# bastienjossen/DDL25Spring

Hardware: AMD Instinct MI355X
Metric: FedAvg rounds/sec + local samples/sec, ResNet-18 CIFAR-10-shape, 8 clients (higher is better)
Workload: dtype fp32; 1 GPU; model=resnet18-cifar10, global_batch=800, parallelism=fedavg-8clients-dp1, clients=8, local_batch=100, local_epochs=1, samples_per_client=6250, client_slots_per_gpu=8, hip_graphs=True, fp32_conv_math=auto

## Files before the change

### csrc/kernels/conv_f32.hip

```cpp
#include "conv_f32_core.h"
#include <cstdlib>

#ifndef F32_PREFETCH
#define F32_PREFETCH 2
#endif

constexpr int FBK = 16;

__device__ __forceinline__ int fswz(int row) { return (row >> 2) & 2; }
__device__ __forceinline__ int lds_off(int row, int ch) { return row * 16 + ((ch ^ fswz(row)) << 2); }

__device__ __forceinline__ int x6_off(int row, int ch, int half) {
  const int f = row & 2;
  const int g = (row ^ (row >> 2)) & 1;
  return row * 32 + 8 * (ch ^ f) + 4 * (half ^ g);
}

template <int MODE, int BP, int BQ, int X6>
__global__ __launch_bounds__(256, (X6 && BP * BQ <= 64 * 128) ? 3 : 2) void convf32_kernel(ConvF32Args a) {
  constexpr int WP = BP / 2, WQ = BQ / 2, TP = WP / 16, TQ = WQ / 16;
  constexpr int RW = X6 ? 32 : 16;
  constexpr int SP = BP * RW, SQ = BQ * RW;
  constexpr int UPK = BP / 64, UQK = BQ / 64;
  constexpr int KUP = BP / 64, KUQ = BQ / 64;
  __shared__ float4 smem4[(2 * (SP + SQ)) / 4];
  float* smem = (float*)smem4;
  __shared__ float xform[2 * 512];

  const int tid = threadIdx.x, lane = tid & 63, wid = tid >> 6, wp = wid >> 1, wq = wid & 1;
  const int gx = gridDim.x, gy = gridDim.y, gz = gridDim.z;
  const int lin = blockIdx.x + gx * (blockIdx.y + gy * blockIdx.z);
  const int u = xcd_remap(lin, gx * gy * gz);
  const int bx = u % gx, by = (u / gx) % gy, g = u / (gx * gy);
  const FGeo o = fgeo<MODE, BP, BQ>(a, bx, by, g, gy);
  const bool split_store = a.split_k > 1;
  if (o.q0 >= o.Qd || o.p0 >= o.Pd) {
    if (!split_store || (a.tickets && o.split == 0)) fzero_slot<MODE, BP>(a, o);
    return;
  }
  const int nk = (o.Kr + FBK - 1) / FBK;
  const int per = (nk + o.nsplit - 1) / o.nsplit;
  const int kt0 = o.split * per, kt1 = min(nk, kt0 + per);

  const int H = a.H, W = a.W, C = a.C, K = a.K, S = a.S, P = a.P, Q = a.Q, st = a.stride, pd = a.pad;
  const float* X = a.x + (long long)g * a.x_gs;
  const float* Wt = a.w + (long long)g * a.w_gs;
  const float* DY = a.dy + (long long)g * a.dy_gs;
  const bool xf = (MODE != F_DGRAD) && a.in_scale != nullptr;
  if (xf) {
    for (int i = tid; i < C; i += 256) {
      xform[i] = a.in_scale[(long long)g * C + i];
      xform[512 + i] = a.in_shift[(long long)g * C + i];
    }
  }
  const bool xrelu = a.in_relu != 0;

  int pk_row[UPK], pk_ch[UPK];
  int pm_rg = 0, pm_kp = 0;
  if constexpr (MODE == F_FWD) {
#pragma unroll
    for (int i = 0; i < UPK; ++i) {
      const int uu = tid + 256 * i;
      pk_row[i] = uu >> 2;
      pk_ch[i] = uu & 3;
    }
  } else {
    pm_kp = tid % (16 / KUP);
    pm_rg = tid / (16 / KUP);
  }
  int qk_row[UQK], qk_ch[UQK], qk_n[UQK], qk_hb[UQK], qk_wb[UQK];
  int qm_rg = 0, qm_kp = 0, qm_r = 0, qm_s = 0, qm_c = 0;
  bool qm_ok = false;
  float qm_sc[4] = {1.f, 1.f, 1.f, 1.f}, qm_sh[4] = {0.f, 0.f, 0.f, 0.f};
  if constexpr (MODE != F_WGRAD) {
    const FDiv dpq = mk_fdiv((uint32_t)(MODE == F_FWD ? P * Q : o.Hs * o.Ws));
    const FDiv dq = mk_fdiv((uint32_t)(MODE == F_FWD ? Q : o.Ws));
    const int PQ = MODE == F_FWD ? P * Q : o.Hs * o.Ws, QQ = MODE == F_FWD ? Q : o.Ws;
#pragma unroll
    for (int i = 0; i < UQK; ++i) {
      const int uu = tid + 256 * i;
      qk_row[i] = uu >> 2;
      qk_ch[i] = uu & 3;
      const int q = o.q0 + qk_row[i];
      if (q < o.Qd) {
        const int n = fdv(q, dpq), rem = q - n * PQ;
        const int y = fdv(rem, dq), xq = rem - y * QQ;
        qk_n[i] = n;
        if (MODE == F_FWD) {
          qk_hb[i] = y * st - pd;
          qk_wb[i] = xq * st - pd;
        } else {
          qk_hb[i] = (o.nph == 4 ? 2 * y + o.pa : y) + pd;
          qk_wb[i] = (o.nph == 4 ? 2 * xq + o.pb : xq) + pd;
        }
      } else {
        qk_n[i] = -1;
        qk_hb[i] = qk_wb[i] = 0;
      }
    }
  } else {
    qm_kp = tid % (16 / KUQ);
    qm_rg = tid / (16 / KUQ);
    const int q = o.q0 + 4 * qm_rg;
    qm_ok = q < o.Qd;
    if (qm_ok) {
      const int tap = q / C;
      qm_c = q - tap * C;
      qm_r = tap / S;
      qm_s = tap - qm_r * S;
    }
  }
  if (xf) __syncthreads();
  if constexpr (MODE == F_WGRAD) {
    if (xf && qm_ok) {
#pragma unroll
      for (int v = 0; v < 4; ++v) { qm_sc[v] = xform[qm_c + v]; qm_sh[v] = xform[512 + qm_c + v]; }
    }
  }
  const FDiv dpix = mk_fdiv((uint32_t)(P * Q)), dpq1 = mk_fdiv((uint32_t)Q);

  constexpr unsigned OOB = 0xFFFFFFF0u;
  const __amdgpu_buffer_rsrc_t rX = __builtin_amdgcn_make_buffer_rsrc(
      (void*)X, 0, (int)((long long)a.N * H * W * C * 4), 0x00020000);
  const __amdgpu_buffer_rsrc_t rW = __builtin_amdgcn_make_buffer_rsrc(
      (void*)Wt, 0, (int)((long long)K * a.R * S * C * 4), 0x00020000);
  const __amdgpu_buffer_rsrc_t rD = __builtin_amdgcn_make_buffer_rsrc(
      (void*)DY, 0, (int)((long long)a.N * P * Q * K * 4), 0x00020000);
  auto bload = [&](const __amdgpu_buffer_rsrc_t& rs, unsigned off) -> float4 {
    const auto v = __builtin_amdgcn_raw_buffer_load_b128(rs, off, 0, 0);
    return __builtin_bit_cast(float4, v);
  };
  constexpr int PF = F32_PREFETCH;
  float4 rpA[2], rqA[2], rpB[2], rqB[2], rpC[2], rqC[2];
  bool qvA[2] = {false, false}, qvB[2] = {false, false}, qvC[2] = {false, false};
  auto load_step = [&](int kt, float4 (&rp)[2], float4 (&rq)[2], bool (&qv)[2]) {
    const int kk0 = kt * FBK;
    if constexpr (MODE == F_FWD) {
#pragma unroll
      for (int i = 0; i < UPK; ++i) {
        const int p = o.p0 + pk_row[i];
        rp[i] = bload(rW, p < o.Pd ? (unsigned)(p * o.Kr + kk0 + 4 * pk_ch[i]) * 4u : OOB);
      }
    } else if constexpr (MODE == F_DGRAD) {
      const int tap = kk0 / K, k0 = kk0 - tap * K;
      const int ir = tap / o.Sn, is = tap - ir * o.Sn;
      const int r = o.r0 + (st == 2 ? 2 : 1) * ir, s = o.s0 + (st == 2 ? 2 : 1) * is;
      const int c = o.p0 + 4 * pm_rg;
#pragma unroll
      for (int j = 0; j < KUP; ++j) {
        const int k = k0 + pm_kp * KUP + j;
        rp[j] = bload(rW, c < C ? (unsigned)(((k * a.R + r) * S + s) * C + c) * 4u : OOB);
      }
    } else {
      const int kch = o.p0 + 4 * pm_rg;
#pragma unroll
      for (int j = 0; j < KUP; ++j) {
        const int pix = kk0 + pm_kp * KUP + j;
        rp[j] = bload(rD, (pix < o.Kr && kch < K) ? (unsigned)(pix * K + kch) * 4u : OOB);
      }
    }
    if constexpr (MODE == F_FWD) {
      const int tap = kk0 / C, c0 = kk0 - tap * C;
      const int r = tap / S, s = tap - r * S;
#pragma unroll
      for (int i = 0; i < UQK; ++i) {
        const int h = qk_hb[i] + r, w = qk_wb[i] + s;
        const bool ok = qk_n[i] >= 0 && (unsigned)h < (unsigned)H && (unsigned)w < (unsigned)W;
        qv[i] = ok;
        rq[i] = bload(rX, ok ? (unsigned)(((qk_n[i] * H + h) * W + w) * C + c0 + 4 * qk_ch[i]) * 4u : OOB);
      }
    } else if constexpr (MODE == F_DGRAD) {
      const int tap = kk0 / K, k0 = kk0 - tap * K;
      const int ir = tap / o.Sn, is = tap - ir * o.Sn;
      const int r = o.r0 + (st == 2 ? 2 : 1) * ir, s = o.s0 + (st == 2 ? 2 : 1) * is;
#pragma unroll
      for (int i = 0; i < UQK; ++i) {
        int ho = qk_hb[i] - r, wo = qk_wb[i] - s;
        bool hit = true;
        if (st == 2) {
          ho >>= 1;
          wo >>= 1;
        } else if (st > 2) {
          hit = ho >= 0 && wo >= 0 && ho % st == 0 && wo % st == 0;
          ho /= st;
          wo /= st;
        }
        const bool ok = hit && qk_n[i] >= 0 && (unsigned)ho < (unsigned)P && (unsigned)wo < (unsigned)Q;
        rq[i] = bload(rD, ok ? (unsigned)(((qk_n[i] * P + ho) * Q + wo) * K + k0 + 4 * qk_ch[i]) * 4u : OOB);
      }
    } else {
#pragma unroll
      for (int j = 0; j < KUQ; ++j) {
        const int pix = kk0 + qm_kp * KUQ + j;
        const int n = fdv(pix, dpix), rem = pix - n * P * Q;
        const int ho = fdv(rem, dpq1), wo = rem - ho * Q;
        const int h = ho * st - pd + qm_r, w = wo * st - pd + qm_s;
        const bool ok = qm_ok && pix < o.Kr && (unsigned)h < (unsigned)H && (unsigned)w < (unsigned)W;
        qv[j] = ok;
        rq[j] = bload(rX, ok ? (unsigned)(((n * H + h) * W + w) * C + qm_c) * 4u : OOB);
      }
    }
  };
  auto xform4 = [&](float4 v, const float* sc, const float* sh) {
    v.x = v.x * sc[0] + sh[0];
    v.y = v.y * sc[1] + sh[1];
    v.z = v.z * sc[2] + sh[2];
    v.w = v.w * sc[3] + sh[3];
    if (xrelu) { v.x = fmaxf(v.x, 0.f); v.y = fmaxf(v.y, 0.f); v.z = fmaxf(v.z, 0.f); v.w = fmaxf(v.w, 0.f); }
    return v;
  };
  auto store_mn = [&](float* img, int rg, int kp, int KU, const float4* v) {
#pragma unroll
    for (int j4 = 0; j4 < 4; ++j4) {
      const int row = 4 * rg + j4;
      const int kk = kp * KU;
      float* d = img + row * 16 + (((kk >> 2) ^ fswz(row)) << 2) + (kk & 3);
      const float e0 = j4 == 0 ? v[0].x : j4 == 1 ? v[0].y : j4 == 2 ? v[0].z : v[0].w;
      if (KU == 2) {
        const float e1 = j4 == 0 ? v[1].x : j4 == 1 ? v[1].y : j4 == 2 ? v[1].z : v[1].w;
        *(float2*)d = make_float2(e0, e1);
      } else {
        *d = e0;
      }
    }
  };
  auto store_k6 = [&](float* img, int row, int ch, float4 v) {
    s4v h, m, l;
    split3(v, h, m, l);
    *(s8v*)(img + x6_off(row, ch, 0)) = cat44(h, m);
    *(s8v*)(img + x6_off(row, ch, 1)) = cat44(l, h);
  };
  auto store_mn6 = [&](float* img, int rg, int kp, int KU, const float4* v) {
#pragma unroll
    for (int j4 = 0; j4 < 4; ++j4) {
      const int row = 4 * rg + j4;
      const int kk = kp * KU, ch = kk >> 2, pos = kk & 3;
      uint16_t* h0 = (uint16_t*)(img + x6_off(row, ch, 0)) + pos;
      uint16_t* h1 = (uint16_t*)(img + x6_off(row, ch, 1)) + pos;
      const float e0 = j4 == 0 ? v[0].x : j4 == 1 ? v[0].y : j4 == 2 ? v[0].z : v[0].w;
      uint16_t ah, am, al;
      split1(e0, ah, am, al);
      if (KU == 2) {
        const float e1 = j4 == 0 ? v[1].x : j4 == 1 ? v[1].y : j4 == 2 ? v[1].z : v[1].w;
        uint16_t bh, bm, bl;
        split1(e1, bh, bm, bl);
        *(uint32_t*)h0 = (uint32_t)ah | ((uint32_t)bh << 16);
        *(uint32_t*)(h0 + 4) = (uint32_t)am | ((uint32_t)bm << 16);
        *(uint32_t*)h1 = (uint32_t)al | ((uint32_t)bl << 16);
        *(uint32_t*)(h1 + 4) = (uint32_t)ah | ((uint32_t)bh << 16);
      } else {
        h0[0] = ah;
        h0[4] = am;
        h1[0] = al;
        h1[4] = ah;
      }
    }
  };
  auto store_step = [&](int buf, int kt, float4 (&rp)[2], float4 (&rq)[2], const bool (&qv)[2]) {
    float* Ps = smem + buf * (SP + SQ);
    float* Qs = Ps + SP;
    if constexpr (MODE == F_FWD) {
#pragma unroll
      for (int i = 0; i < UPK; ++i) {
        if constexpr (X6) store_k6(Ps, pk_row[i], pk_ch[i], rp[i]);
        else *(float4*)(Ps + lds_off(pk_row[i], pk_ch[i])) = rp[i];
      }
    } else {
      if constexpr (X6) store_mn6(Ps, pm_rg, pm_kp, KUP, rp);
      else store_mn(Ps, pm_rg, pm_kp, KUP, rp);
    }
    if constexpr (MODE == F_FWD) {
      if (xf) {
        const int kk0 = kt * FBK, c0 = kk0 - (kk0 / C) * C;
#pragma unroll
        for (int i = 0; i < UQK; ++i) {
          const int c = c0 + 4 * qk_ch[i];
          if (qv[i]) rq[i] = xform4(rq[i], xform + c, xform + 512 + c);
        }
      }
    } else if constexpr (MODE == F_WGRAD) {
      if (xf) {
#pragma unroll
        for (int j = 0; j < KUQ; ++j)
          if (qv[j]) rq[j] = xform4(rq[j], qm_sc, qm_sh);
      }
    }
    if constexpr (MODE != F_WGRAD) {
#pragma unroll
      for (int i = 0; i < UQK; ++i) {
        if constexpr (X6) store_k6(Qs, qk_row[i], qk_ch[i], rq[i]);
        else *(float4*)(Qs + lds_off(qk_row[i], qk_ch[i])) = rq[i];
      }
    } else {
      if constexpr (X6) store_mn6(Qs, qm_rg, qm_kp, KUQ, rq);
      else store_mn(Qs, qm_rg, qm_kp, KUQ, rq);
    }
  };

  f4v acc[TP][TQ];
#pragma unroll
  for (int i = 0; i < TP; ++i)
#pragma unroll
    for (int j = 0; j < TQ; ++j) acc[i][j] = (f4v){0.f, 0.f, 0.f, 0.f};

  auto step = [&](int kt, float4 (&cp)[2], float4 (&cq)[2], bool (&cv)[2], float4 (&np)[2],
                  float4 (&nq)[2], bool (&nv)[2]) {
    const int cur = (kt - kt0) & 1;
    if (kt + PF < kt1) load_step(kt + PF, np, nq, nv);
    const float* Ps = smem + cur * (SP + SQ);
    const float* Qs = Ps + SP;
    if constexpr (X6) {
      s8v a0[TP], a1[TP], b0[TQ], b1[TQ];
#pragma unroll
      for (int ti = 0; ti < TP; ++ti) {
        const int R = wp * WP + ti * 16 + (lane & 15);
        a0[ti] = *(const s8v*)(Ps + x6_off(R, lane >> 4, 0));
        a1[ti] = *(const s8v*)(Ps + x6_off(R, lane >> 4, 1));
      }
#pragma unroll
      for (int tj = 0; tj < TQ; ++tj) {
        const int R = wq * WQ + tj * 16 + (lane & 15);
        b0[tj] = *(const s8v*)(Qs + x6_off(R, lane >> 4, 0));
        b1[tj] = *(const s8v*)(Qs + x6_off(R, lane >> 4, 1));
      }
#pragma unroll
      for (int ti = 0; ti < TP; ++ti)
#pragma unroll
        for (int tj = 0; tj < TQ; ++tj) {
          f4v c = __builtin_amdgcn_mfma_f32_16x16x32_bf16(a1[ti], b0[tj], (f4v){0.f, 0.f, 0.f, 0.f}, 0, 0, 0);
          c = __builtin_amdgcn_mfma_f32_16x16x32_bf16(a0[ti], b1[tj], c, 0, 0, 0);
          c = __builtin_amdgcn_mfma_f32_16x16x32_bf16(a0[ti], b0[tj], c, 0, 0, 0);
#pragma unroll
          for (int v = 0; v < 4; ++v) acc[ti][tj][v] = acc[ti][tj][v] + c[v];
        }
    } else {
      float4 af[TP], bfr[TQ];
#pragma unroll
      for (int ti = 0; ti < TP; ++ti)
        af[ti] = *(const float4*)(Ps + lds_off(wp * WP + ti * 16 + (lane & 15), lane >> 4));
#pragma unroll
      for (int tj = 0; tj < TQ; ++tj)
        bfr[tj] = *(const float4*)(Qs + lds_off(wq * WQ + tj * 16 + (lane & 15), lane >> 4));
#pragma unroll
      for (int s4 = 0; s4 < 4; ++s4)
#pragma unroll
        for (int ti = 0; ti < TP; ++ti)
#pragma unroll
          for (int tj = 0; tj < TQ; ++tj) {
            const float av = s4 == 0 ? af[ti].x : s4 == 1 ? af[ti].y : s4 == 2 ? af[ti].z : af[ti].w;
            const float bv = s4 == 0 ? bfr[tj].x : s4 == 1 ? bfr[tj].y : s4 == 2 ? bfr[tj].z : bfr[tj].w;
            acc[ti][tj] = __builtin_amdgcn_mfma_f32_16x16x4f32(av, bv, acc[ti][tj], 0, 0, 0);
          }
    }
    if (kt + 1 < kt1) store_step(cur ^ 1, kt + 1, cp, cq, cv);
    __syncthreads();
  };
  if (kt0 < kt1) {
    load_step(kt0, rpA, rqA, qvA);
    if (kt0 + 1 < kt1) load_step(kt0 + 1, rpB, rqB, qvB);
    if constexpr (PF == 3) {
      if (kt0 + 2 < kt1) load_step(kt0 + 2, rpC, rqC, qvC);
    }
    store_step(0, kt0, rpA, rqA, qvA);
    __syncthreads();
    if constexpr (PF == 3) {
      for (int kt = kt0; kt < kt1; kt += 3) {
        step(kt, rpB, rqB, qvB, rpA, rqA, qvA);
        if (kt + 1 < kt1) step(kt + 1, rpC, rqC, qvC, rpB, rqB, qvB);
        if (kt + 2 < kt1) step(kt + 2, rpA, rqA, qvA, rpC, rqC, qvC);
      }
    } else {
      for (int kt = kt0; kt < kt1; kt += 2) {
        step(kt, rpB, rqB, qvB, rpA, rqA, qvA);
        if (kt + 1 < kt1) step(kt + 1, rpA, rqA, qvA, rpB, rqB, qvB);
      }
    }
  }

  if (split_store) {
#pragma unroll
    for (int ti = 0; ti < TP; ++ti)
#pragma unroll
      for (int tj = 0; tj < TQ; ++tj) {
        const int q = o.q0 + wq * WQ + tj * 16 + (lane & 15);
        const int p = o.p0 + wp * WP + ti * 16 + 4 * (lane >> 4);
        if (q >= o.Qd || p >= o.Pd) continue;
        if constexpr (MODE == F_WGRAD) {
          float* d = a.partial + ((long long)o.split * a.G + g) * o.Pd * o.Qd;
#pragma unroll
          for (int v = 0; v < 4; ++v)
            if (p + v < o.Pd) d[(long long)(p + v) * o.Qd + q] = acc[ti][tj][v];
        } else {
          const long long qmax = (long long)a.slots / o.nph * BQ;
          float* d = a.partial + (((long long)o.split * a.G + g) * o.nph + o.phase) * qmax * o.Pd;
          *(float4*)(d + (long long)q * o.Pd + p) = make_float4(acc[ti][tj][0], acc[ti][tj][1],
                                                                acc[ti][tj][2], acc[ti][tj][3]);
        }
      }
    if (a.tickets) {
      __threadfence();
      __syncthreads();
      int* const last = (int*)smem;
      int* const ticket = a.tickets + ((long long)g * o.nph + o.phase) * gx + bx;
      if (tid == 0) *last = atomicAdd(ticket, 1) == o.nsplit - 1;
      __syncthreads();
      if (!*last) return;
      __threadfence();
      if constexpr (MODE != F_WGRAD) {
        const long long qmax = (long long)a.slots / o.nph * BQ;
        const long long slice = (long long)a.G * o.nph * qmax * o.Pd;
        const float* base = a.partial + ((long long)g * o.nph + o.phase) * qmax * o.Pd;
#pragma unroll
        for (int ti = 0; ti < TP; ++ti)
#pragma unroll
          for (int tj = 0; tj < TQ; ++tj) {
            const int q = o.q0 + wq * WQ + tj * 16 + (lane & 15);
            const int p = o.p0 + wp * WP + ti * 16 + 4 * (lane >> 4);
            f4v sm = (f4v){0.f, 0.f, 0.f, 0.f};
            if (q < o.Qd && p < o.Pd) {
              const float* src = base + (long long)q * o.Pd + p;
              for (int k = 0; k < o.nsplit; ++k) {
                const float4 v = *(const float4*)(src + k * slice);
                sm[0] += v.x; sm[1] += v.y; sm[2] += v.z; sm[3] += v.w;
              }
            }
            acc[ti][tj] = sm;
          }
        __syncthreads();
        if (tid == 0) *ticket = 0;
        fepi<MODE, BP, BQ, Lay16<BP, BQ>>(a, o, acc, smem);
        return;
      } else {
        const long long per = (long long)o.Pd * o.Qd;
        const float* src = a.partial + (long long)g * per;
        float* dst = a.out + (long long)g * a.out_gs;
        for (int e = tid; e < BP * (BQ / 4); e += 256) {
          const int p = o.p0 + e / (BQ / 4), q = o.q0 + 4 * (e % (BQ / 4));
          if (p >= o.Pd || q >= o.Qd) continue;
          const long long off = (long long)p * o.Qd + q;
          float4 sum = make_float4(0.f, 0.f, 0.f, 0.f);
          for (int k = 0; k < o.nsplit; ++k) {
            const float4 v = *(const float4*)(src + (long long)k * a.G * per + off);
            sum.x += v.x; sum.y += v.y; sum.z += v.z; sum.w += v.w;
          }
          float4 b = a.accumulate ? *(const float4*)(dst + off) : make_float4(0.f, 0.f, 0.f, 0.f);
          b.x += a.gscale * sum.x; b.y += a.gscale * sum.y; b.z += a.gscale * sum.z; b.w += a.gscale * sum.w;
          *(float4*)(dst + off) = b;
        }
        if (tid == 0) *ticket = 0;
      }
    }
    return;
  }
  fepi<MODE, BP, BQ, Lay16<BP, BQ>>(a, o, acc, smem);
}

template <int V>
__global__ __launch_bounds__(256) void convf32_wgrad_reduce(const float* __restrict__ part, float* out,
                                                            long long out_gs, int G, long long nv,
                                                            int splits, int accumulate, float gscale) {
  typedef float vec __attribute__((ext_vector_type(V)));
  const long long per = nv * V;
  GSTRIDE_LOOP(t, (long long)G * nv) {
    const long long g = t / nv, i = (t - g * nv) * V;
    vec s = (vec)(0.f);
    const float* src = part + g * per + i;
    const long long sstride = (long long)G * per;
    int k = 0;
    for (; k + 8 <= splits; k += 8) {
      vec v[8];
#pragma unroll
      for (int j = 0; j < 8; ++j) v[j] = *(const vec*)(src + (long long)(k + j) * sstride);
#pragma unroll
      for (int j = 0; j < 8; ++j) s += v[j];
    }
    for (; k < splits; ++k) s += *(const vec*)(src + (long long)k * sstride);
    float* d = out + g * out_gs + i;
    vec b = accumulate ? *(const vec*)d : (vec)(0.f);
    b += gscale * s;
    *(vec*)d = b;
  }
}

static void launch_wgrad_reduce(const float* part, float* out, long long out_gs, int G, long long n, int splits,
                                int accumulate, float gscale, hipStream_t s) {
  static const long long v4_min = [] {
    const char* e = getenv("DDL_WGRAD_REDUCE_V4_MIN");
    return e ? atoll(e) : 512LL * 256;
  }();
  if ((long long)G * (n / 4) >= v4_min)
    hipLaunchKernelGGL(convf32_wgrad_reduce<4>, dim3(grid_for((long long)G * (n / 4), 256)), dim3(256), 0, s, part,
                       out, out_gs, G, n / 4, splits, accumulate, gscale);
  else
    hipLaunchKernelGGL(convf32_wgrad_reduce<1>, dim3(grid_for((long long)G * n, 256)), dim3(256), 0, s, part, out,
                       out_gs, G, n, splits, accumulate, gscale);
}

DDL_API int ddl_convf32_wgrad_reduce(const float* part, float* out, long long out_gs, int G, long long n, int splits,
                                     int accumulate, float gscale, hipStream_t s) {
  if (n % 4) return (int)hipErrorInvalidValue;
  launch_wgrad_reduce(part, out, out_gs, G, n, splits, accumulate, gscale, s);
  return (int)hipGetLastError();
}

static void fdims(const ConvF32Args& a, int mode, long long& Pd, long long& Qd, long long& Qmax, long long& Kr,
                  int& nph) {
  nph = (mode == F_DGRAD && a.stride == 2) ? 4 : 1;
  if (mode == F_FWD) { Pd = a.K; Qd = Qmax = (long long)a.N * a.P * a.Q; Kr = (long long)a.R * a.S * a.C; }
  else if (mode == F_DGRAD) {
    Pd = a.C;
    const int Hs = nph == 4 ? (a.H + 1) >> 1 : a.H, Ws = nph == 4 ? (a.W + 1) >> 1 : a.W;
    Qd = Qmax = (long long)a.N * Hs * Ws;
    Kr = (long long)a.R * a.S * a.K;
  } else { Pd = a.K; Qd = Qmax = (long long)a.R * a.S * a.C; Kr = (long long)a.N * a.P * a.Q; }
}

DDL_API long long ddl_convf32_slots(const ConvF32Args* ap, int mode, int cfg) {
  long long Pd, Qd, Qmax, Kr;
  int nph;
  fdims(*ap, mode, Pd, Qd, Qmax, Kr, nph);
  const int bq = ((cfg >> 8) & 0xff) * 16;
  if (bq <= 0) return -1;
  return nph * ((Qmax + bq - 1) / bq);
}

DDL_API long long ddl_convf32_workspace(const ConvF32Args* ap, int mode, int cfg) {
  if (ap->split_k <= 1) return 0;
  long long Pd, Qd, Qmax, Kr;
  int nph;
  fdims(*ap, mode, Pd, Qd, Qmax, Kr, nph);
  const int bq = ((cfg >> 8) & 0xff) * 16;
  if (mode == F_WGRAD) return (long long)ap->split_k * ap->G * Pd * Qd;
  const long long qm = (Qmax + bq - 1) / bq * bq;
  return (long long)ap->split_k * ap->G * nph * qm * Pd;
}

template <int MODE, int BP, int BQ, int X6>
static int launch_tile(ConvF32Args a, hipStream_t s) {
  long long Pd, Qd, Qmax, Kr;
  int nph;
  fdims(a, MODE, Pd, Qd, Qmax, Kr, nph);
  const long long ntp = (Pd + BP - 1) / BP, ntq = (Qmax + BQ - 1) / BQ;
  a.slots = (int)(nph * ntq);
  const int split = a.split_k < 1 ? 1 : a.split_k;
  a.split_k = split;
  if (split > 1) {
    const long long need = MODE == F_WGRAD ? (long long)split * a.G * Pd * Qd
                                           : (long long)split * a.G * nph * ntq * BQ * Pd;
    if (!a.partial || need > a.partial_cap) return (int)hipErrorInvalidValue;
  }
  const dim3 grid((unsigned)(ntp * ntq), (unsigned)(nph * split), (unsigned)a.G);
  if (split == 1 || (long long)a.G * nph * ntp * ntq > a.tickets_cap) a.tickets = nullptr;
  hipLaunchKernelGGL((convf32_kernel<MODE, BP, BQ, X6>), grid, dim3(256), 0, s, a);
  hipError_t e = hipGetLastError();
  if (e != hipSuccess || split == 1 || a.tickets) return (int)e;
  if (MODE == F_WGRAD) {
    launch_wgrad_reduce((const float*)a.partial, a.out, a.out_gs, a.G, Pd * Qd, split, a.accumulate, a.gscale, s);
  } else {
    hipLaunchKernelGGL((convf32_splitk_epilogue<MODE, BP, BQ>), dim3((unsigned)(ntp * ntq), nph, a.G),
                       dim3(256), 0, s, a);
  }
  return (int)hipGetLastError();
}

template <int MODE, int X6>
static int launch_math(const ConvF32Args& a, int bp, int bq, hipStream_t s) {
  if (bp == 64 && bq == 64) return launch_tile<MODE, 64, 64, X6>(a, s);
  if (bp == 64 && bq == 128) return launch_tile<MODE, 64, 128, X6>(a, s);
  if (bp == 128 && bq == 64) return launch_tile<MODE, 128, 64, X6>(a, s);
  if (bp == 128 && bq == 128) return launch_tile<MODE, 128, 128, X6>(a, s);
  return (int)hipErrorInvalidValue;
}

template <int MODE>
static int launch_mode(const ConvF32Args& a, int cfg, hipStream_t s) {
  const int bp = (cfg & 0xff) * 16, bq = ((cfg >> 8) & 0xff) * 16;
  return (cfg >> 16) & 1 ? launch_math<MODE, 1>(a, bp, bq, s) : launch_math<MODE, 0>(a, bp, bq, s);
}

DDL_API int ddl_convf32(const ConvF32Args* ap, int mode, int cfg, hipStream_t s) {
  const ConvF32Args& a = *ap;
  if (a.G < 1 || a.N < 1 || a.C < 1 || a.K < 1 || a.stride < 1) return (int)hipErrorInvalidValue;
  if (a.C > 512 && a.in_scale) return (int)hipErrorInvalidValue;
  const long long lim = (1LL << 31) - 64;
  if ((long long)a.N * a.H * a.W * a.C * 4 > lim || (long long)a.K * a.R * a.S * a.C * 4 > lim ||
      (long long)a.N * a.P * a.Q * a.K * 4 > lim)
    return (int)hipErrorInvalidValue;
  if (mode == F_FWD) {
    if (a.C % 16 || a.K % 4) return (int)hipErrorInvalidValue;
    return launch_mode<F_FWD>(a, cfg, s);
  }
  if (mode == F_DGRAD) {
    if (a.K % 16 || a.C % 4) return (int)hipErrorInvalidValue;
    return launch_mode<F_DGRAD>(a, cfg, s);
  }
  if (mode == F_WGRAD) {
    if (a.C % 4 || a.K % 4) return (int)hipErrorInvalidValue;
    if (!a.accumulate && a.gscale != 1.f) return (int)hipErrorInvalidValue;
    return launch_mode<F_WGRAD>(a, cfg, s);
  }
  return (int)hipErrorInvalidValue;
}

DDL_API int ddl_convf32_args_size() { return (int)sizeof(ConvF32Args); }
```

### ddl25spring_amd/ops/functional_f32.py

```python
from __future__ import annotations

import ctypes
import math
import os

import torch

from . import _lib
from . import workspace as ws
from ._lib import check, ptr, stream

F_FWD, F_DGRAD, F_WGRAD = 0, 1, 2
WS_CAP = 1 << 26
_WS: dict = {}
TARGET_WG = int(os.environ.get("DDL_F32_TARGET_WG", "640"))


def is_f32(t) -> bool:
    return t is not None and t.is_cuda and t.dtype == torch.float32


class SlotStats:
    __slots__ = ("t", "rows")

    def __init__(self):
        self.t = None
        self.rows = 0


def workspace(device, role: str = "main") -> torch.Tensor:
    key = f"{device}:{role}"
    b = _WS.get(key)
    if b is None:
        if torch.cuda.is_current_stream_capturing():
            raise RuntimeError("fp32 split-K workspace first requested inside a graph capture: run one eager "
                               "step (or functional_f32.ensure_workspace) before capturing")
        ensure_workspace(device)
        b = _WS[key]
    return b


def ensure_workspace(device) -> None:
    for role in ("main", "side"):
        key = f"{device}:{role}"
        if key not in _WS:
            _WS[key] = torch.empty(WS_CAP, dtype=torch.float32, device=device)
            _WS[key + ":tickets"] = torch.zeros(TICKETS_CAP, dtype=torch.int32, device=device)
    if torch.device(device).type == "cuda" and _dev_key(device) not in _TICKETS:
        _TICKETS[_dev_key(device)] = torch.zeros(TICKETS_N, dtype=torch.int32, device=device)


TICKETS_CAP = 1 << 18
WG_FOLD = [os.environ.get("DDL_F32_WG_FOLD", "0") == "1"]


def _dims(mode, g):
    if mode == F_FWD:
        return g.K, g.N * g.P * g.Q, g.R * g.S * g.C, 1
    if mode == F_DGRAD:
        if g.stride == 2:
            hs, wsz = (g.H + 1) // 2, (g.W + 1) // 2
            rn, sn = (g.R + 1) // 2, (g.S + 1) // 2
            return g.C, g.N * hs * wsz, rn * sn * g.K, 4
        return g.C, g.N * g.H * g.W, g.R * g.S * g.K, 1
    return g.K, g.R * g.S * g.C, g.N * g.P * g.Q, 1


def cfg_of(bp: int, bq: int) -> int:
    return (bp // 16) | ((bq // 16) << 8)


MATHS = ("mfma32", "x6", "auto")
_MATH = [os.environ.get("DDL_F32_MATH", "auto")]
if _MATH[0] not in MATHS:
    raise ValueError(f"DDL_F32_MATH={_MATH[0]!r}: expected one of {MATHS}")


def math() -> str:
    return _MATH[0]


def set_math(name: str) -> None:
    if name not in MATHS:
        raise ValueError(f"fp32 conv math {name!r}: expected one of {MATHS}")
    if name != _MATH[0]:
        _MATH[0] = name
        _PLANS.clear()


X6_BIT = 1 << 16
HALO_BIT = 1 << 17
_HALO = [os.environ.get("DDL_F32_HALO", "1") != "0"]
HALO_HPMAX = 288


def set_halo(on: bool) -> None:
    if bool(on) != _HALO[0]:
        _HALO[0] = bool(on)
        _PLANS.clear()


HALO_MIN_W = int(os.environ.get("DDL_F32_HALO_MIN_W", "4"))
HALO_PADW = [os.environ.get("DDL_F32_HALO_PADW", "1") != "0"]


def halo_ok(mode: int, g, auto: bool = False) -> bool:
    if mode not in (F_FWD, F_DGRAD) or g.stride != 1 or g.R != g.S or g.R not in (1, 3) or g.pad != (g.R - 1) // 2:
        return False
    if g.P != g.H or g.Q != g.W:
        return False
    OH, OWr = g.P, g.Q
    if OWr < 4 or OWr > 128:
        return False
    if auto and OWr < HALO_MIN_W:
        return False
    OW = 1 << (OWr - 1).bit_length()
    if OW != OWr and (not HALO_PADW[0] or (auto and g.R == 1)):
        return False
    TR = 128 // OW
    if TR <= OH:
        if OH % TR:
            return False
        SR = TR
    else:
        if TR % OH:
            return False
        SR = OH
    HP = (TR // SR) * (SR + g.R - 1) * (OW + g.S - 1)
    SC, Pd = (g.C, g.K) if mode == F_FWD else (g.K, g.C)
    if not (HP <= HALO_HPMAX and SC % 16 == 0 and Pd % 4 == 0):
        return False
    return _x6h_native_ok(mode, g)


_X6H_OK: dict = {}


def _x6h_native_ok(mode: int, g) -> bool:
    key = (mode, g)
    r = _X6H_OK.get(key)
    if r is None:
        try:
            lib = _lib.kernels()
        except Exception:
            return True
        a = _args(g)
        r = bool(lib.ddl_x6h_ok(ctypes.byref(a), mode, cfg_of(64, 128)))
        _X6H_OK[key] = r
    return r


HALO_TINY, HALO_SMALL, HALO_LARGE = 26624, 32768, 45056


def halo_layout(mode: int, geom, bp: int = 64):
    out = (ctypes.c_int * 5)()
    a = _args(geom)
    if _lib.kernels().ddl_x6h_layout(ctypes.byref(a), mode, cfg_of(bp, 128), out) != 0:
        return None
    return dict(zip(("ROWB", "SEGB", "HBYTES", "HP", "tier"), out))


def halo_residency(mode: int, bp: int, rs: int, tier: int, padw: bool = False) -> int:
    return int(_lib.kernels().ddl_x6h_residency(mode, bp, rs, tier, int(padw)))


_FLAT_ENV = os.environ.get("DDL_F32_FLAT1X1", "fd")
FLAT1X1 = [_FLAT_ENV != "0", "fdw" if _FLAT_ENV == "1" else _FLAT_ENV]


def _launch_geom(geom, mode: str = "f"):
    if not FLAT1X1[0] or mode not in FLAT1X1[1] or geom.R != 1 or geom.S != 1 or geom.stride != 1 or geom.pad != 0:
        return geom
    if geom.W & (geom.W - 1) == 0 and geom.W <= 128:
        return geom
    npix = geom.N * geom.H * geom.W
    if npix % 128:
        return geom
    return type(geom)(geom.G, 1, npix // 128, 128, geom.C, geom.K, 1, 1, 1, 0)


def _cfg(cfg: int) -> int:
    if _MATH[0] == "x6":
        return cfg | X6_BIT
    if _MATH[0] == "mfma32":
        return cfg & ~X6_BIT
    return cfg


_PLANS: dict = {}
_OVERRIDE: dict = {}
_MODE_NAMES = ("fwd", "dgrad", "wgrad")
_TUNED_PATH = os.path.join(os.path.dirname(os.path.abspath(__file__)), "f32_plans.json")
_TUNED: dict | None = None


def _tuned(mode: int, g):
    global _TUNED
    if _TUNED is None:
        _TUNED = {}
        if os.environ.get("DDL_F32_TUNED", "1") != "0" and os.path.exists(_TUNED_PATH):
            import json
            with open(_TUNED_PATH) as f:
                _TUNED = json.load(f).get("plans", {})
    key = f"{_MODE_NAMES[mode]}:{g.G},{g.N},{g.H},{g.W},{g.C},{g.K},{g.R},{g.S},{g.stride},{g.pad}"
    if _MATH[0] == "auto":
        p = _TUNED.get(f"auto:{key}")
        if p is not None:
            return cfg_of(p[0], p[1]) | (X6_BIT if p[3] == "x6" else 0), int(p[2])
        p = _TUNED.get(f"x6:{key}")
        return None if p is None else (cfg_of(p[0], p[1]) | X6_BIT, int(p[2]))
    if _MATH[0] != "mfma32":
        key = f"{_MATH[0]}:{key}"
    p = _TUNED.get(key)
    return None if p is None else (cfg_of(p[0], p[1]), int(p[2]))


BLAS = [os.environ.get("DDL_F32_BLAS", "0")]


def vendor_gemm(mode: int, g) -> bool:
    if BLAS[0] in ("0", "1"):
        return BLAS[0] == "1"
    _tuned(mode, g)
    return f"blas:{_MODE_NAMES[mode]}:{g.G},{g.N},{g.H},{g.W},{g.C},{g.K},{g.R},{g.S},{g.stride},{g.pad}" in _TUNED


def set_plan(mode: int, geom, bp: int, bq: int, split: int, engine: str | None = None) -> None:
    bits = {None: X6_BIT, "x6": X6_BIT, "x6h": X6_BIT | HALO_BIT, "mfma32": 0}[engine]
    _OVERRIDE[(mode, geom)] = (cfg_of(bp, bq) | bits, int(split))
    _PLANS.pop((mode, geom), None)


def clear_plan(mode: int, geom) -> None:
    _OVERRIDE.pop((mode, geom), None)
    _PLANS.pop((mode, geom), None)


_RECORD_PATH = os.environ.get("DDL_F32_RECORD", "")
_RECORDED: set = set()


def _write_record():
    import json
    rows = sorted({(m, (g.G, g.N, g.H, g.W, g.C, g.K, g.R, g.S, g.stride, g.pad)) for m, g in _RECORDED})
    with open(_RECORD_PATH, "w") as f:
        json.dump([{"mode": _MODE_NAMES[m], "geom": list(g)} for m, g in rows], f)


if _RECORD_PATH:
    import atexit
    atexit.register(_write_record)


def plan(mode: int, geom) -> tuple[int, int]:
    key = (mode, geom)
    p = _PLANS.get(key)
    if p is not None:
        return p
    if _RECORD_PATH:
        _RECORDED.add(key)
    p = _OVERRIDE.get(key)
    if p is None and _HALO[0] and _MATH[0] != "mfma32" and halo_ok(mode, geom, auto=True):
        p = _halo_plan(mode, geom)
    if p is None:
        p = _tuned(mode, geom)
    if p is None:
        Pd, Qd, Kr, nph = _dims(mode, geom)
        bp = 128 if Pd > 64 else 64
        bq = 128 if Qd > 64 else 64
        tiles = -(-Pd // bp) * -(-Qd // bq) * nph * geom.G
        nk = -(-Kr // 16)
        split = 1
        while tiles * split < TARGET_WG and nk >= split * 2 * 8 and split < 64:
            split *= 2
        p = (cfg_of(bp, bq) | X6_BIT, split)
    _PLANS[key] = p
    return p


def _halo_plan(mode: int, geom) -> tuple[int, int]:
    _tuned(mode, geom)
    if TARGET_WG != 1:
        p = _TUNED.get(f"x6h:{_MODE_NAMES[mode]}:{geom.G},{geom.N},{geom.H},{geom.W},{geom.C},{geom.K},"
                       f"{geom.R},{geom.S},{geom.stride},{geom.pad}")
        if p is not None:
            return cfg_of(int(p[0]), int(p[1])) | X6_BIT | HALO_BIT, int(p[2])
    Pd, Qd, _, _ = _dims(mode, geom)
    SC = geom.C if mode == F_FWD else geom.K
    bp = 128 if Pd > 64 and geom.Q > 4 else 64
    tiles = -(-Pd // bp) * -(-Qd // 128) * geom.G
    nch = SC // 16
    split = 1
    padded = geom.Q & (geom.Q - 1) != 0
    while not padded and tiles * split < TARGET_WG and nch >= split * 2 * 4 and split < 32:
        split *= 2
    return cfg_of(bp, 128) | X6_BIT | HALO_BIT, split


def _args(geom, **kw) -> _lib.ConvF32Args:
    a = _lib.ConvF32Args()
    a.gscale = 1.0
    for k, v in kw.items():
        setattr(a, k, v)
    a.G, a.N, a.H, a.W, a.C, a.K = geom.G, geom.N, geom.H, geom.W, geom.C, geom.K
    a.R, a.S, a.P, a.Q, a.stride, a.pad = geom.R, geom.S, geom.P, geom.Q, geom.stride, geom.pad
    return a


def _gs(t) -> int:
    return 0 if t is None else t.stride(0)


def _launch(a, mode: int, geom, device, split_k: int = 0, ws_role: str = "main") -> None:
    lib = _lib.kernels()
    cfg, split = plan(mode, geom)
    if split_k:
        split = split_k
    a.split_k = split
    cfg = _cfg(cfg)
    if cfg & HALO_BIT and not halo_ok(mode, geom):
        cfg &= ~HALO_BIT
    if split > 1:
        need = lib.ddl_convf32_workspace(ctypes.byref(a), mode, cfg)
        buf = workspace(device, ws_role)
        if need > buf.numel():
            a.split_k = split = 1
        else:
            a.partial, a.partial_cap = buf.data_ptr(), buf.numel()
            if WG_FOLD[0] and not (cfg & HALO_BIT):
                t = _WS[f"{device}:{ws_role}:tickets"]
                a.tickets, a.tickets_cap = t.data_ptr(), t.numel()
    name = ("conv_fwd", "conv_dgrad", "conv_wgrad")[mode] + "_f32"
    if cfg & HALO_BIT:
        ws_buf = split_weights(a, mode, geom, device)
        a.wsplit, a.ws_gs = ws_buf.data_ptr(), ws_buf.stride(0)
        check(lib.ddl_x6h(ctypes.byref(a), mode, cfg & ~HALO_BIT, stream()), name + "_halo")
        return
    check(lib.ddl_convf32(ctypes.byref(a), mode, cfg, stream()), name)


def split_weights(a, mode: int, geom, device) -> torch.Tensor:
    T = geom.R * geom.S
    layout = 0 if mode == F_FWD else 1
    scope = _PRESPLIT[0]
    if scope is not None:
        key = (int(a.w), layout, geom.G, geom.K, T, geom.C, int(a.w_gs))
        buf = scope.lookup(key)
        if buf is not None:
            return buf
    out = torch.empty(geom.G, geom.K * T * geom.C * 6, dtype=torch.uint8, device=device)
    check(_lib.kernels().ddl_x6_split_weights(a.w, out.data_ptr(), geom.G, geom.K, T, geom.C, 0 if mode == F_FWD else 1,
                                              a.w_gs, out.stride(0), 0, stream()), "x6_split_weights")
    return out


class _SplitDesc(ctypes.Structure):
    _fields_ = [("w", ctypes.c_void_p), ("out", ctypes.c_void_p), ("w_gs", ctypes.c_longlong),
                ("o_gs", ctypes.c_longlong), ("G", ctypes.c_int), ("K", ctypes.c_int), ("T", ctypes.c_int),
                ("C", ctypes.c_int), ("layout", ctypes.c_int), ("blk0", ctypes.c_int), ("nblk", ctypes.c_int),
                ("pad_", ctypes.c_int)]


_PRESPLIT: list = [None]
PRESPLIT = [os.environ.get("DDL_F32_PRESPLIT", "1") != "0"]
PRESPLIT_SIDE = [os.environ.get("DDL_F32_PRESPLIT_SIDE", "0") == "1"]
PRESPLIT_HEAD_FRAC = float(os.environ.get("DDL_F32_PRESPLIT_HEAD", "0.05"))
_SPLIT_STREAMS: dict = {}


class PresplitScope:

    def __init__(self):
        self.keys: list = []
        self._seen: set = set()
        self.bufs: dict = {}
        self.tables: list = []
        self.tail: set = set()
        self._pending = None
        self.state = "record"
        self._prev = None

    def lookup(self, key):
        if self.state == "ready":
            if self._pending is not None and key in self.tail:
                torch.cuda.current_stream().wait_event(self._pending)
                self._pending = None
            return self.bufs.get(key)
        if key not in self._seen:
            self._seen.add(key)
            self.keys.append(key)
        return None

    def __enter__(self):
        self._prev = _PRESPLIT[0]
        if not PRESPLIT[0]:
            return self
        if self.state == "ready":
            lib = _lib.kernels()
            desc, n, nb = self.tables[0]
            check(lib.ddl_x6_split_weights_multi(ptr(desc), n, nb, stream()), "x6_split_weights_multi")
            if len(self.tables) > 1:
                cur = torch.cuda.current_stream()
                side = _SPLIT_STREAMS.get(cur.device)
                if side is None:
                    side = _SPLIT_STREAMS[cur.device] = torch.cuda.Stream(device=cur.device)
                side.wait_stream(cur)
                desc, n, nb = self.tables[1]
                with torch.cuda.stream(side):
                    check(lib.ddl_x6_split_weights_multi(ptr(desc), n, nb, stream()), "x6_split_weights_multi")
                    ev = torch.cuda.Event()
                    ev.record(side)
                self._pending = ev
        _PRESPLIT[0] = self
        return self

    def __exit__(self, *exc):
        _PRESPLIT[0] = self._prev
        if self._pending is not None:
            torch.cuda.current_stream().wait_event(self._pending)
            self._pending = None
        if self.state == "record" and self.keys and not torch.cuda.is_current_stream_capturing() \
                and exc[0] is None:
            self._build()
        return False

    def _build(self):
        lib = _lib.kernels()
        if lib.ddl_x6_split_desc_size() != ctypes.sizeof(_SplitDesc):
            raise RuntimeError("ABI mismatch for SplitDesc")
        dev = torch.device("cuda", torch.cuda.current_device())
        vol = [k[2] * k[3] * k[4] * k[5] for k in self.keys]
        nhead = len(self.keys)
        if PRESPLIT_SIDE[0] and len(self.keys) > 1:
            nhead, acc = 1, vol[0]
            while nhead < len(self.keys) and acc + vol[nhead] <= PRESPLIT_HEAD_FRAC * sum(vol):
                acc += vol[nhead]
                nhead += 1
        self.tail = set(self.keys[nhead:])
        self.tables = []
        for part in (self.keys[:nhead], self.keys[nhead:]):
            if not part:
                continue
            descs = (_SplitDesc * len(part))()
            blk = 0
            for i, key in enumerate(part):
                w, layout, G, K, T, C, w_gs = key
                buf = torch.empty(G, K * T * C * 6, dtype=torch.uint8, device=dev)
                self.bufs[key] = buf
                nblk = max(1, min(1024, -(-G * K * T * C // 16 // 256)))
                d = descs[i]
                d.w, d.out, d.w_gs, d.o_gs = w, buf.data_ptr(), w_gs, buf.stride(0)
                d.G, d.K, d.T, d.C, d.layout, d.blk0, d.nblk = G, K, T, C, layout, blk, nblk
                blk += nblk
            raw = torch.frombuffer(bytearray(bytes(descs)), dtype=torch.uint8)
            self.tables.append((raw.to(dev), len(part), blk))
        self.state = "ready"


def _store_identity(owner):
    store = getattr(owner, "store", None)
    data = getattr(store, "data", None)
    if data is None:
        return None
    return data.data_ptr(), data.numel(), id(data.untyped_storage())


def presplit_scope(owner) -> "PresplitScope | contextlib.nullcontext":
    sig = _store_identity(owner)
    sc = getattr(owner, "_f32_presplit", None)
    if sc is None or getattr(owner, "_f32_presplit_sig", None) != sig:
        sc = PresplitScope()
        owner._f32_presplit = sc
        owner._f32_presplit_sig = sig
    return sc


def _slots(a, mode: int, geom) -> int:
    cfg, _ = plan(mode, geom)
    if uses_halo(mode, geom):
        return int(_lib.kernels().ddl_x6h_slots(ctypes.byref(a), mode))
    return int(_lib.kernels().ddl_convf32_slots(ctypes.byref(a), mode, _cfg(cfg)))


def slot_rows(mode: int, geom) -> int:
    cfg, _ = plan(mode, geom)
    bq = ((_cfg(cfg) >> 8) & 0xFF) * 16
    if uses_halo(mode, geom) and geom.Q & (geom.Q - 1):
        return bq // (1 << (geom.Q - 1).bit_length()) * geom.Q
    return bq
# ... 384 lines not shown
```

Baseline: 42270 samples/s.

## Stage dgrad/wgrad MN operands as bf16 split planes read via transpose LDS loads

For the X6 (three-way bf16 split) path in dgrad and wgrad, operands loaded along the reduction dimension are now stored in LDS as separate hi/mid/lo bf16 planes with a swizzled layout. They are then read back with ds_read_b64_tr_b16 transposing loads instead of the per-row x6 layout. The global-load thread mapping is changed to match, and partial lgkmcnt waits let MFMAs start before all fragment reads finish. The aim is to cut LDS bank conflicts and register shuffling in the MN staging. It adds inline asm that depends on the hardware and a new template dimension, and it is on by default through a cfg bit set from Python.

```diff
diff --git a/csrc/kernels/conv_f32.hip b/csrc/kernels/conv_f32.hip
--- a/csrc/kernels/conv_f32.hip
+++ b/csrc/kernels/conv_f32.hip
@@ -16,11 +16,46 @@
   return row * 32 + 8 * (ch ^ f) + 4 * (half ^ g);
 }
 
-template <int MODE, int BP, int BQ, int X6>
+template <int B>
+__device__ __forceinline__ int pl_off(int k, int quad) {
+  const int sw = B >= 128 ? 2 * (k & 7) : 2 * ((k >> 1) & 3);
+  return k * (B * 2) + (((quad >> 1) ^ sw) << 4) + ((quad & 1) << 3);
+}
+__device__ __forceinline__ unsigned lds_base(const void* p) {
+  return (unsigned)(size_t)(const __attribute__((address_space(3))) char*)p;
+}
+template <int OFF>
+__device__ __forceinline__ i2v lds_rdtr(unsigned addr) {
+  i2v r;
+  asm volatile("ds_read_b64_tr_b16 %0, %1 offset:%2" : "=v"(r) : "v"(addr), "i"(OFF) : "memory");
+  return r;
+}
+__device__ __forceinline__ void lgkm_wait_le(int n) {
+  if (n == 12) asm volatile("s_waitcnt lgkmcnt(12)" ::: "memory");
+  else if (n == 8) asm volatile("s_waitcnt lgkmcnt(8)" ::: "memory");
+  else if (n == 4) asm volatile("s_waitcnt lgkmcnt(4)" ::: "memory");
+  else asm volatile("s_waitcnt lgkmcnt(0)" ::: "memory");
+  __builtin_amdgcn_sched_barrier(0);
+}
+struct PlFrag { i4v lh, hm; };
+template <int V>
+struct IConst { static constexpr int value = V; };
+template <int B>
+__device__ __forceinline__ PlFrag pl_read(unsigned ad) {
+  constexpr int PL = 16 * B * 2;
+  const i2v l = lds_rdtr<2 * PL>(ad), h1 = lds_rdtr<0>(ad), h2 = lds_rdtr<0>(ad), m = lds_rdtr<PL>(ad);
+  PlFrag f;
+  f.lh = (i4v){l.x, l.y, h1.x, h1.y};
+  f.hm = (i4v){h2.x, h2.y, m.x, m.y};
+  return f;
+}
+
+template <int MODE, int BP, int BQ, int X6, int MNP>
 __global__ __launch_bounds__(256, (X6 && BP * BQ <= 64 * 128) ? 3 : 2) void convf32_kernel(ConvF32Args a) {
   constexpr int WP = BP / 2, WQ = BQ / 2, TP = WP / 16, TQ = WQ / 16;
   constexpr int RW = X6 ? 32 : 16;
-  constexpr int SP = BP * RW, SQ = BQ * RW;
+  constexpr bool PLP = X6 && MNP && MODE != F_FWD, PLQ = X6 && MNP && MODE == F_WGRAD;
+  constexpr int SP = BP * (PLP ? 24 : RW), SQ = BQ * (PLQ ? 24 : RW);
   constexpr int UPK = BP / 64, UQK = BQ / 64;
   constexpr int KUP = BP / 64, KUQ = BQ / 64;
   __shared__ float4 smem4[(2 * (SP + SQ)) / 4];
@@ -65,8 +100,8 @@
       pk_ch[i] = uu & 3;
     }
   } else {
-    pm_kp = tid % (16 / KUP);
-    pm_rg = tid / (16 / KUP);
+    pm_kp = PLP ? tid / (BP / 4) : tid % (16 / KUP);
+    pm_rg = PLP ? tid % (BP / 4) : tid / (16 / KUP);
   }
   int qk_row[UQK], qk_ch[UQK], qk_n[UQK], qk_hb[UQK], qk_wb[UQK];
   int qm_rg = 0, qm_kp = 0, qm_r = 0, qm_s = 0, qm_c = 0;
@@ -99,8 +134,8 @@
       }
     }
   } else {
-    qm_kp = tid % (16 / KUQ);
-    qm_rg = tid / (16 / KUQ);
+    qm_kp = PLQ ? tid / (BQ / 4) : tid % (16 / KUQ);
+    qm_rg = PLQ ? tid % (BQ / 4) : tid / (16 / KUQ);
     const int q = o.q0 + 4 * qm_rg;
     qm_ok = q < o.Qd;
     if (qm_ok) {
@@ -148,14 +183,14 @@
       const int c = o.p0 + 4 * pm_rg;
 #pragma unroll
       for (int j = 0; j < KUP; ++j) {
-        const int k = k0 + pm_kp * KUP + j;
+        const int k = k0 + (PLP ? pm_kp + j * (16 / KUP) : pm_kp * KUP + j);
         rp[j] = bload(rW, c < C ? (unsigned)(((k * a.R + r) * S + s) * C + c) * 4u : OOB);
       }
     } else {
       const int kch = o.p0 + 4 * pm_rg;
 #pragma unroll
       for (int j = 0; j < KUP; ++j) {
-        const int pix = kk0 + pm_kp * KUP + j;
+        const int pix = kk0 + (PLP ? pm_kp + j * (16 / KUP) : pm_kp * KUP + j);
         rp[j] = bload(rD, (pix < o.Kr && kch < K) ? (unsigned)(pix * K + kch) * 4u : OOB);
       }
     }
@@ -191,7 +226,7 @@
     } else {
 #pragma unroll
       for (int j = 0; j < KUQ; ++j) {
-        const int pix = kk0 + qm_kp * KUQ + j;
+        const int pix = kk0 + (PLQ ? qm_kp + j * (16 / KUQ) : qm_kp * KUQ + j);
         const int n = fdv(pix, dpix), rem = pix - n * P * Q;
         const int ho = fdv(rem, dpq1), wo = rem - ho * Q;
         const int h = ho * st - pd + qm_r, w = wo * st - pd + qm_s;
@@ -256,6 +291,19 @@
       }
     }
   };
+  auto store_pl = [&](float* img, auto bc, int rg, int kp, int KU, const float4* v) {
+    constexpr int B = decltype(bc)::value;
+#pragma unroll
+    for (int j = 0; j < 2; ++j) {
+      if (j >= KU) continue;
+      s4v h, m, l;
+      split3(v[j], h, m, l);
+      char* d = (char*)img + pl_off<B>(kp + j * (16 / KU), rg);
+      *(s4v*)d = h;
+      *(s4v*)(d + 32 * B) = m;
+      *(s4v*)(d + 64 * B) = l;
+    }
+  };
   auto store_step = [&](int buf, int kt, float4 (&rp)[2], float4 (&rq)[2], const bool (&qv)[2]) {
     float* Ps = smem + buf * (SP + SQ);
     float* Qs = Ps + SP;
@@ -266,7 +314,8 @@
         else *(float4*)(Ps + lds_off(pk_row[i], pk_ch[i])) = rp[i];
       }
     } else {
-      if constexpr (X6) store_mn6(Ps, pm_rg, pm_kp, KUP, rp);
+      if constexpr (PLP) store_pl(Ps, IConst<BP>{}, pm_rg, pm_kp, KUP, rp);
+      else if constexpr (X6) store_mn6(Ps, pm_rg, pm_kp, KUP, rp);
       else store_mn(Ps, pm_rg, pm_kp, KUP, rp);
     }
     if constexpr (MODE == F_FWD) {
@@ -292,10 +341,24 @@
         else *(float4*)(Qs + lds_off(qk_row[i], qk_ch[i])) = rq[i];
       }
     } else {
-      if constexpr (X6) store_mn6(Qs, qm_rg, qm_kp, KUQ, rq);
+      if constexpr (PLQ) store_pl(Qs, IConst<BQ>{}, qm_rg, qm_kp, KUQ, rq);
+      else if constexpr (X6) store_mn6(Qs, qm_rg, qm_kp, KUQ, rq);
       else store_mn(Qs, qm_rg, qm_kp, KUQ, rq);
     }
   };
+
+  unsigned pfa[TP], qfa[TQ];
+  if constexpr (PLP) {
+    const unsigned b0 = lds_base(smem);
+#pragma unroll
+    for (int ti = 0; ti < TP; ++ti)
+      pfa[ti] = b0 + pl_off<BP>(4 * (lane >> 4) + ((lane >> 2) & 3), (wp * WP + ti * 16) / 4 + (lane & 3));
+    if constexpr (PLQ) {
+#pragma unroll
+      for (int tj = 0; tj < TQ; ++tj)
+        qfa[tj] = b0 + SP * 4 + pl_off<BQ>(4 * (lane >> 4) + ((lane >> 2) & 3), (wq * WQ + tj * 16) / 4 + (lane & 3));
+    }
+  }
 
   f4v acc[TP][TQ];
 #pragma unroll
@@ -311,28 +374,58 @@
     const float* Qs = Ps + SP;
     if constexpr (X6) {
       s8v a0[TP], a1[TP], b0[TQ], b1[TQ];
-#pragma unroll
-      for (int ti = 0; ti < TP; ++ti) {
-        const int R = wp * WP + ti * 16 + (lane & 15);
-        a0[ti] = *(const s8v*)(Ps + x6_off(R, lane >> 4, 0));
-        a1[ti] = *(const s8v*)(Ps + x6_off(R, lane >> 4, 1));
-      }
-#pragma unroll
-      for (int tj = 0; tj < TQ; ++tj) {
-        const int R = wq * WQ + tj * 16 + (lane & 15);
-        b0[tj] = *(const s8v*)(Qs + x6_off(R, lane >> 4, 0));
-        b1[tj] = *(const s8v*)(Qs + x6_off(R, lane >> 4, 1));
-      }
-#pragma unroll
-      for (int ti = 0; ti < TP; ++ti)
+      const unsigned bufb = (unsigned)(cur * (SP + SQ) * 4);
+      if constexpr (PLP) {
+#pragma unroll
+        for (int ti = 0; ti < TP; ++ti) {
+          const PlFrag f = pl_read<BP>(pfa[ti] + bufb);
+          a0[ti] = __builtin_bit_cast(s8v, f.hm);
+          a1[ti] = __builtin_bit_cast(s8v, f.lh);
+        }
+      } else {
+#pragma unroll
+        for (int ti = 0; ti < TP; ++ti) {
+          const int R = wp * WP + ti * 16 + (lane & 15);
+          a0[ti] = *(const s8v*)(Ps + x6_off(R, lane >> 4, 0));
+          a1[ti] = *(const s8v*)(Ps + x6_off(R, lane >> 4, 1));
+        }
+      }
+      if constexpr (PLQ) {
 #pragma unroll
         for (int tj = 0; tj < TQ; ++tj) {
-          f4v c = __builtin_amdgcn_mfma_f32_16x16x32_bf16(a1[ti], b0[tj], (f4v){0.f, 0.f, 0.f, 0.f}, 0, 0, 0);
-          c = __builtin_amdgcn_mfma_f32_16x16x32_bf16(a0[ti], b1[tj], c, 0, 0, 0);
-          c = __builtin_amdgcn_mfma_f32_16x16x32_bf16(a0[ti], b0[tj], c, 0, 0, 0);
-#pragma unroll
-          for (int v = 0; v < 4; ++v) acc[ti][tj][v] = acc[ti][tj][v] + c[v];
-        }
+          const PlFrag f = pl_read<BQ>(qfa[tj] + bufb);
+          b0[tj] = __builtin_bit_cast(s8v, f.hm);
+          b1[tj] = __builtin_bit_cast(s8v, f.lh);
+        }
+      } else {
+#pragma unroll
+        for (int tj = 0; tj < TQ; ++tj) {
+          const int R = wq * WQ + tj * 16 + (lane & 15);
+          b0[tj] = *(const s8v*)(Qs + x6_off(R, lane >> 4, 0));
+          b1[tj] = *(const s8v*)(Qs + x6_off(R, lane >> 4, 1));
+        }
+      }
+      auto tile = [&](int ti, int tj) {
+        f4v c = __builtin_amdgcn_mfma_f32_16x16x32_bf16(a1[ti], b0[tj], (f4v){0.f, 0.f, 0.f, 0.f}, 0, 0, 0);
+        c = __builtin_amdgcn_mfma_f32_16x16x32_bf16(a0[ti], b1[tj], c, 0, 0, 0);
+        c = __builtin_amdgcn_mfma_f32_16x16x32_bf16(a0[ti], b0[tj], c, 0, 0, 0);
+#pragma unroll
+        for (int v = 0; v < 4; ++v) acc[ti][tj][v] = acc[ti][tj][v] + c[v];
+      };
+      if constexpr (PLQ) {
+#pragma unroll
+        for (int tj = 0; tj < TQ; ++tj) {
+          lgkm_wait_le(4 * (TQ - 1 - tj));
+#pragma unroll
+          for (int ti = 0; ti < TP; ++ti) tile(ti, tj);
+        }
+      } else {
+        if constexpr (PLP) lgkm_wait_le(0);
+#pragma unroll
+        for (int ti = 0; ti < TP; ++ti)
+#pragma unroll
+          for (int tj = 0; tj < TQ; ++tj) tile(ti, tj);
+      }
     } else {
       float4 af[TP], bfr[TQ];
 #pragma unroll
@@ -535,7 +628,7 @@
   return (long long)ap->split_k * ap->G * nph * qm * Pd;
 }
 
-template <int MODE, int BP, int BQ, int X6>
+template <int MODE, int BP, int BQ, int X6, int MNP>
 static int launch_tile(ConvF32Args a, hipStream_t s) {
   long long Pd, Qd, Qmax, Kr;
   int nph;
@@ -551,7 +644,7 @@
   }
   const dim3 grid((unsigned)(ntp * ntq), (unsigned)(nph * split), (unsigned)a.G);
   if (split == 1 || (long long)a.G * nph * ntp * ntq > a.tickets_cap) a.tickets = nullptr;
-  hipLaunchKernelGGL((convf32_kernel<MODE, BP, BQ, X6>), grid, dim3(256), 0, s, a);
+  hipLaunchKernelGGL((convf32_kernel<MODE, BP, BQ, X6, MNP>), grid, dim3(256), 0, s, a);
   hipError_t e = hipGetLastError();
   if (e != hipSuccess || split == 1 || a.tickets) return (int)e;
   if (MODE == F_WGRAD) {
@@ -563,19 +656,23 @@
   return (int)hipGetLastError();
 }
 
-template <int MODE, int X6>
+template <int MODE, int X6, int MNP>
 static int launch_math(const ConvF32Args& a, int bp, int bq, hipStream_t s) {
-  if (bp == 64 && bq == 64) return launch_tile<MODE, 64, 64, X6>(a, s);
-  if (bp == 64 && bq == 128) return launch_tile<MODE, 64, 128, X6>(a, s);
-  if (bp == 128 && bq == 64) return launch_tile<MODE, 128, 64, X6>(a, s);
-  if (bp == 128 && bq == 128) return launch_tile<MODE, 128, 128, X6>(a, s);
+  if (bp == 64 && bq == 64) return launch_tile<MODE, 64, 64, X6, MNP>(a, s);
+  if (bp == 64 && bq == 128) return launch_tile<MODE, 64, 128, X6, MNP>(a, s);
+  if (bp == 128 && bq == 64) return launch_tile<MODE, 128, 64, X6, MNP>(a, s);
+  if (bp == 128 && bq == 128) return launch_tile<MODE, 128, 128, X6, MNP>(a, s);
   return (int)hipErrorInvalidValue;
 }
 
 template <int MODE>
 static int launch_mode(const ConvF32Args& a, int cfg, hipStream_t s) {
   const int bp = (cfg & 0xff) * 16, bq = ((cfg >> 8) & 0xff) * 16;
-  return (cfg >> 16) & 1 ? launch_math<MODE, 1>(a, bp, bq, s) : launch_math<MODE, 0>(a, bp, bq, s);
+  if (!((cfg >> 16) & 1)) return launch_math<MODE, 0, 0>(a, bp, bq, s);
+  if constexpr (MODE != F_FWD) {
+    if ((cfg >> 18) & 1) return launch_math<MODE, 1, 1>(a, bp, bq, s);
+  }
+  return launch_math<MODE, 1, 0>(a, bp, bq, s);
 }
 
 DDL_API int ddl_convf32(const ConvF32Args* ap, int mode, int cfg, hipStream_t s) {
diff --git a/ddl25spring_amd/ops/functional_f32.py b/ddl25spring_amd/ops/functional_f32.py
--- a/ddl25spring_amd/ops/functional_f32.py
+++ b/ddl25spring_amd/ops/functional_f32.py
@@ -89,6 +89,26 @@
 
 
 X6_BIT = 1 << 16
+MN_PLANES_BIT = 1 << 18
+MN_STAGES = ("planes", "regs")
+_MN_DEFAULT = {F_DGRAD: "planes", F_WGRAD: "planes"}
+_MN_ENV = os.environ.get("DDL_F32_MN_STAGE", "")
+if _MN_ENV not in ("",) + MN_STAGES:
+    raise ValueError(f"DDL_F32_MN_STAGE={_MN_ENV!r}: expected one of {MN_STAGES}")
+_MN_STAGE = {m: (_MN_ENV or d) for m, d in _MN_DEFAULT.items()}
+
+
+def mn_stage(mode: int = F_WGRAD) -> str:
+    return _MN_STAGE[mode]
+
+
+def set_mn_stage(name: str | None, mode: int | None = None) -> None:
+    if name is not None and name not in MN_STAGES:
+        raise ValueError(f"fp32 conv MN staging {name!r}: expected one of {MN_STAGES}")
+    for m in (F_DGRAD, F_WGRAD) if mode is None else (mode,):
+        _MN_STAGE[m] = name or _MN_DEFAULT[m]
+
+
 HALO_BIT = 1 << 17
 _HALO = [os.environ.get("DDL_F32_HALO", "1") != "0"]
 HALO_HPMAX = 288
@@ -180,7 +200,11 @@
     return type(geom)(geom.G, 1, npix // 128, 128, geom.C, geom.K, 1, 1, 1, 0)
 
 
-def _cfg(cfg: int) -> int:
+def _cfg(cfg: int, mode: int | None = None) -> int:
+    if mode is not None:
+        cfg &= ~MN_PLANES_BIT
+        if _MN_STAGE.get(mode) == "planes":
+            cfg |= MN_PLANES_BIT
     if _MATH[0] == "x6":
         return cfg | X6_BIT
     if _MATH[0] == "mfma32":
@@ -318,7 +342,7 @@
     if split_k:
         split = split_k
     a.split_k = split
-    cfg = _cfg(cfg)
+    cfg = _cfg(cfg, mode)
     if cfg & HALO_BIT and not halo_ok(mode, geom):
         cfg &= ~HALO_BIT
     if split > 1:
@@ -335,7 +359,7 @@
     if cfg & HALO_BIT:
         ws_buf = split_weights(a, mode, geom, device)
         a.wsplit, a.ws_gs = ws_buf.data_ptr(), ws_buf.stride(0)
-        check(lib.ddl_x6h(ctypes.byref(a), mode, cfg & ~HALO_BIT, stream()), name + "_halo")
+        check(lib.ddl_x6h(ctypes.byref(a), mode, cfg & ~(HALO_BIT | MN_PLANES_BIT), stream()), name + "_halo")
         return
     check(lib.ddl_convf32(ctypes.byref(a), mode, cfg, stream()), name)
 
```

Result: no change. 42510 samples/s, median of 6 (+0.6%).
